# liuQuan98/GCL

Hardware: AMD Instinct MI355X
Metric: active voxels/sec thru ResUNetBN2C fwd+bwd+GCL loss, KITTI 0.3m (higher is better)
Workload: dtype f32; 1 GPU; configs[2]: GCL training step (finest_contrastive_loss), ResUNetBN2C-32 conv1 k=5, KITTI-shaped ray-cast clouds @0.3 m, bs=4 x 7 clouds per GPU, positive groups 'fixed16'; global_batch=4, parallelism=dp1

## Files before the change

gcl_amd/csrc/norm.hip:

```cpp
#include "common.h"

namespace gcl {

static inline int bn_rows_per_wg(long long n, int c) {
  int rows = 1024;
  while (rows > 64 && n / rows < 1024) rows >>= 1;
  (void)c;
  return rows;
}

__device__ __forceinline__ float4 mask_as_y(const unsigned long long* __restrict__ mask, long long e) {
  const unsigned long long* m = mask + (e >> 6) * 4;
  const int b = (int)(e & 63);
  return make_float4((float)((m[0] >> b) & 1), (float)((m[1] >> b) & 1), (float)((m[2] >> b) & 1),
                     (float)((m[3] >> b) & 1));
}

template <bool BWD>
__global__ void __launch_bounds__(256) k_bn_reduce(const float* __restrict__ x, const float* __restrict__ dy,
                                                   const float* __restrict__ y, long long n, int c,
                                                   const float* __restrict__ mean, const float* __restrict__ rstd,
                                                   int relu, const unsigned long long* __restrict__ mask,
                                                   int rows_per_wg, double* partial, int dy_ld = 0, int want_gmax = 0) {
  const long long gld = dy_ld ? dy_ld : c;
  __shared__ double red[2][256][4];
  const int cq_n = c >> 2;
  const int cq = threadIdx.x % cq_n, rl = threadIdx.x / cq_n, rstep = 256 / cq_n;
  const long long r_begin = (long long)blockIdx.x * rows_per_wg;
  long long r_end = r_begin + rows_per_wg;
  if (r_end > n) r_end = n;
  double s0[4] = {0, 0, 0, 0}, s1[4] = {0, 0, 0, 0};
  float gm[4] = {0.f, 0.f, 0.f, 0.f};
  float4 mu = make_float4(0, 0, 0, 0), rs = make_float4(1, 1, 1, 1);
  if (BWD) {
    mu = reinterpret_cast<const float4*>(mean)[cq];
    rs = reinterpret_cast<const float4*>(rstd)[cq];
  }
#define BN_ACC(xv, g, yv)                                                                                     \
  if (!BWD) {                                                                                                 \
    s0[0] += xv.x; s0[1] += xv.y; s0[2] += xv.z; s0[3] += xv.w;                                               \
    s1[0] += (double)xv.x * xv.x; s1[1] += (double)xv.y * xv.y;                                               \
    s1[2] += (double)xv.z * xv.z; s1[3] += (double)xv.w * xv.w;                                               \
  } else {                                                                                                    \
    if (relu) {                                                                                               \
      g.x = yv.x > 0.f ? g.x : 0.f; g.y = yv.y > 0.f ? g.y : 0.f;                                             \
      g.z = yv.z > 0.f ? g.z : 0.f; g.w = yv.w > 0.f ? g.w : 0.f;                                             \
    }                                                                                                         \
    s0[0] += g.x; s0[1] += g.y; s0[2] += g.z; s0[3] += g.w;                                                   \
    gm[0] = fmaxf(gm[0], fabsf(g.x)); gm[1] = fmaxf(gm[1], fabsf(g.y));                                       \
    gm[2] = fmaxf(gm[2], fabsf(g.z)); gm[3] = fmaxf(gm[3], fabsf(g.w));                                       \
    s1[0] += (double)g.x * ((xv.x - mu.x) * rs.x); s1[1] += (double)g.y * ((xv.y - mu.y) * rs.y);             \
    s1[2] += (double)g.z * ((xv.z - mu.z) * rs.z); s1[3] += (double)g.w * ((xv.w - mu.w) * rs.w);             \
  }
  const float4 z4 = make_float4(0, 0, 0, 0);
  long long r = r_begin + rl;
  for (; r + rstep < r_end; r += 2 * rstep) {
    const long long q = r + rstep;
    float4 xa = reinterpret_cast<const float4*>(x + r * c)[cq], xb = reinterpret_cast<const float4*>(x + q * c)[cq];
    float4 ga = z4, gb = z4, ya = z4, yb = z4;
    if (BWD) {
      ga = reinterpret_cast<const float4*>(dy + r * gld)[cq];
      gb = reinterpret_cast<const float4*>(dy + q * gld)[cq];
      if (relu) {
        if (mask) {
          ya = mask_as_y(mask, r * cq_n + cq);
          yb = mask_as_y(mask, q * cq_n + cq);
        } else {
          ya = reinterpret_cast<const float4*>(y + r * c)[cq];
          yb = reinterpret_cast<const float4*>(y + q * c)[cq];
        }
      }
    }
    BN_ACC(xa, ga, ya)
    BN_ACC(xb, gb, yb)
  }
  if (r < r_end) {
    float4 xa = reinterpret_cast<const float4*>(x + r * c)[cq];
    float4 ga = z4, ya = z4;
    if (BWD) {
      ga = reinterpret_cast<const float4*>(dy + r * gld)[cq];
      if (relu) ya = mask ? mask_as_y(mask, r * cq_n + cq) : reinterpret_cast<const float4*>(y + r * c)[cq];
    }
    BN_ACC(xa, ga, ya)
  }
#undef BN_ACC
#pragma unroll
  for (int j = 0; j < 4; ++j) {
    red[0][threadIdx.x][j] = s0[j];
    red[1][threadIdx.x][j] = s1[j];
  }
  __syncthreads();
  if (rl == 0) {
    const long long nwg = gridDim.x;
#pragma unroll
    for (int j = 0; j < 4; ++j) {
      double a = 0, b = 0;
      for (int q = 0; q < rstep; ++q) {
        a += red[0][q * cq_n + cq][j];
        b += red[1][q * cq_n + cq][j];
      }
      partial[(long long)(cq * 4 + j) * nwg + blockIdx.x] = a;
      partial[(long long)(c + cq * 4 + j) * nwg + blockIdx.x] = b;
    }
  }
  if (BWD && want_gmax) {
    __syncthreads();
#pragma unroll
    for (int j = 0; j < 4; ++j) red[0][threadIdx.x][j] = (double)gm[j];
    __syncthreads();
    if (rl == 0) {
      const long long nwg = gridDim.x;
#pragma unroll
      for (int j = 0; j < 4; ++j) {
        double a = 0;
        for (int q = 0; q < rstep; ++q) a = fmax(a, red[0][q * cq_n + cq][j]);
        partial[(long long)(2 * c + cq * 4 + j) * nwg + blockIdx.x] = a;
      }
    }
  }
}

template <typename T>
__device__ __forceinline__ void reduce_runs(const T* __restrict__ p1, const T* __restrict__ p2, int n_part, double& s,
                                            double& ss) {
  __shared__ double red[2][256];
  __shared__ double red2[2][16];
  const int t = threadIdx.x;
  double a0 = 0, a1 = 0, a2 = 0, a3 = 0, b0 = 0, b1 = 0, b2 = 0, b3 = 0;
  int w = t;
  for (; w + 768 < n_part; w += 1024) {
    a0 += (double)p1[w];
    a1 += (double)p1[w + 256];
    a2 += (double)p1[w + 512];
    a3 += (double)p1[w + 768];
    b0 += (double)p2[w];
    b1 += (double)p2[w + 256];
    b2 += (double)p2[w + 512];
    b3 += (double)p2[w + 768];
  }
  for (; w < n_part; w += 256) {
    a0 += (double)p1[w];
    b0 += (double)p2[w];
  }
  red[0][t] = (a0 + a1) + (a2 + a3);
  red[1][t] = (b0 + b1) + (b2 + b3);
  __syncthreads();
  if (t < 32) {
    const int which = t >> 4, g = t & 15;
    double u = 0;
#pragma unroll
    for (int q = 0; q < 16; ++q) u += red[which][g * 16 + q];
    red2[which][g] = u;
  }
  __syncthreads();
  s = 0;
  ss = 0;
  if (t == 0) {
#pragma unroll
    for (int q = 0; q < 16; ++q) {
      s += red2[0][q];
      ss += red2[1][q];
    }
  }
}

__global__ void __launch_bounds__(256) k_bn_stats_final(const double* __restrict__ partial, int nwg, long long n,
                                                        int c, float eps, float momentum, float* running_mean,
                                                        float* running_var, float* mean, float* rstd) {
  const int ch = blockIdx.x;
  double s, ss;
  reduce_runs(partial + (long long)ch * nwg, partial + ((long long)c + ch) * nwg, nwg, s, ss);
  if (threadIdx.x != 0) return;
  double m = s / (double)n;
  double var = ss / (double)n - m * m;
  if (var < 0) var = 0;
  mean[ch] = (float)m;
  rstd[ch] = (float)(1.0 / sqrt(var + (double)eps));
  if (running_mean) {
    double unb = (n > 1) ? var * (double)n / (double)(n - 1) : var;
    running_mean[ch] = (float)((1.0 - momentum) * running_mean[ch] + momentum * m);
    running_var[ch] = (float)((1.0 - momentum) * running_var[ch] + momentum * unb);
  }
}

constexpr int BN_DIRECT_MAX = 1 << 20;
__device__ __forceinline__ void reduce_min_max(const float* __restrict__ p1, const float* __restrict__ p2, int n_part,
                                               float& lo, float& hi) {
  __shared__ float mm[2][256];
  const int t = threadIdx.x;
  float a = 3.0e38f, b = -3.0e38f;
  for (int w = t; w < n_part; w += 256) {
    a = fminf(a, p1[w]);
    b = fmaxf(b, p2[w]);
  }
  mm[0][t] = a;
  mm[1][t] = b;
  __syncthreads();
  for (int o = 128; o > 0; o >>= 1) {
    if (t < o) {
      mm[0][t] = fminf(mm[0][t], mm[0][t + o]);
      mm[1][t] = fmaxf(mm[1][t], mm[1][t + o]);
    }
    __syncthreads();
  }
  lo = mm[0][0];
  hi = mm[1][0];
}

struct BnRange {
  float* xrange;
  const float* weight;
  const float* bias;
  int relu;
  const int* add_amax;
  const int* max_with;
  int* y_amax;
};
__global__ void __launch_bounds__(256) k_bn_stats_direct(const float* __restrict__ partial, int n_part, long long n, int c,
                                                         float eps, float momentum, float* running_mean,
                                                         float* running_var, float* mean, float* rstd, BnRange rg) {
  const int ch = blockIdx.x;
  double s, ss;
  reduce_runs(partial + (long long)ch * n_part, partial + ((long long)c + ch) * n_part, n_part, s, ss);
  float xlo = 0.f, xhi = 0.f;
  if (rg.y_amax)
    reduce_min_max(partial + ((long long)2 * c + ch) * n_part, partial + ((long long)3 * c + ch) * n_part, n_part, xlo, xhi);
  if (threadIdx.x != 0) return;
  double m = s / (double)n;
  double var = ss / (double)n - m * m;
  if (var < 0) var = 0;
  const float mu = (float)m, rs = (float)(1.0 / sqrt(var + (double)eps));
  mean[ch] = mu;
  rstd[ch] = rs;
  if (running_mean) {
    double unb = (n > 1) ? var * (double)n / (double)(n - 1) : var;
    running_mean[ch] = (float)((1.0 - momentum) * running_mean[ch] + momentum * m);
    running_var[ch] = (float)((1.0 - momentum) * running_var[ch] + momentum * unb);
  }
  if (rg.y_amax) {
    if (rg.xrange) {
      rg.xrange[ch] = xlo;
      rg.xrange[c + ch] = xhi;
    }
    const float w = rg.weight[ch], b = rg.bias[ch];
    const float f_lo = (xlo - mu) * rs * w + b, f_hi = (xhi - mu) * rs * w + b;
    float bound = rg.relu ? fmaxf(fmaxf(f_lo, f_hi), 0.f) : fmaxf(fabsf(f_lo), fabsf(f_hi));
    if (rg.add_amax) bound += __int_as_float(amax_slot_bits(rg.add_amax));
    if (rg.max_with) bound = fmaxf(bound, __int_as_float(amax_slot_bits(rg.max_with)));
    amax_slot_publish(rg.y_amax, __float_as_int(bound), (unsigned)ch);
  }
}

struct BnBwdRange {
  const float* xrange;
  const float* mean;
  const float* rstd;
  const float* weight;
  long long n;
  int* dx_amax;
};
__global__ void __launch_bounds__(256) k_bn_bwd_final(const double* __restrict__ partial, int nwg, int c,
                                                      float* sum_g, float* sum_gx, BnBwdRange rg) {
  const int ch = blockIdx.x;
  double s, ss;
  reduce_runs(partial + (long long)ch * nwg, partial + ((long long)c + ch) * nwg, nwg, s, ss);
  double gmax = 0;
  if (rg.dx_amax) {
    __shared__ double gm[256];
    double a = 0;
    const double* p3 = partial + ((long long)2 * c + ch) * nwg;
    for (int w = threadIdx.x; w < nwg; w += 256) a = fmax(a, p3[w]);
    gm[threadIdx.x] = a;
    __syncthreads();
    for (int o = 128; o > 0; o >>= 1) {
      if ((int)threadIdx.x < o) gm[threadIdx.x] = fmax(gm[threadIdx.x], gm[threadIdx.x + o]);
      __syncthreads();
    }
    gmax = gm[0];
  }
  if (threadIdx.x != 0) return;
  sum_g[ch] = (float)s;
  sum_gx[ch] = (float)ss;
  if (rg.dx_amax) {
    const float mu = rg.mean[ch], rs = rg.rstd[ch], inv_n = 1.0f / (float)rg.n;
    const float xh = fmaxf(fabsf(rg.xrange[ch] - mu), fabsf(rg.xrange[c + ch] - mu)) * rs;
    const float bound = fabsf(rg.weight[ch] * rs) * ((float)gmax + fabsf((float)s) * inv_n + xh * fabsf((float)ss) * inv_n);
    amax_slot_publish(rg.dx_amax, __float_as_int(bound * 1.0000153f), (unsigned)ch);
  }
}

__device__ __forceinline__ void publish_amax(float m, int* amax_bits) {
#pragma unroll
  for (int o = 32; o > 0; o >>= 1) m = fmaxf(m, __shfl_xor(m, o));
  __shared__ float wm[4];
  if ((threadIdx.x & 63) == 0) wm[threadIdx.x >> 6] = m;
  __syncthreads();
  if (threadIdx.x == 0) {
    amax_slot_publish(amax_bits, __float_as_int(fmaxf(fmaxf(wm[0], wm[1]), fmaxf(wm[2], wm[3]))), blockIdx.x);
  }
}
__device__ __forceinline__ float amax4(float m, const float4& v) {
  return fmaxf(m, fmaxf(fmaxf(fabsf(v.x), fabsf(v.y)), fmaxf(fabsf(v.z), fabsf(v.w))));
}

struct BnFwdC { float4 mu, rs, wv, bv; };
__device__ __forceinline__ BnFwdC bn_fwd_c(const float* mean, const float* rstd, const float* weight, const float* bias, int cq) {
  BnFwdC k;
  k.mu = reinterpret_cast<const float4*>(mean)[cq]; k.rs = reinterpret_cast<const float4*>(rstd)[cq];
  k.wv = reinterpret_cast<const float4*>(weight)[cq]; k.bv = reinterpret_cast<const float4*>(bias)[cq];
  return k;
}
__device__ __forceinline__ float4 bn_fwd_one(const float4& xv, const float4& rv, bool has_res, int relu, const BnFwdC& k) {
  float4 o;
  o.x = (xv.x - k.mu.x) * k.rs.x * k.wv.x + k.bv.x;
  o.y = (xv.y - k.mu.y) * k.rs.y * k.wv.y + k.bv.y;
  o.z = (xv.z - k.mu.z) * k.rs.z * k.wv.z + k.bv.z;
  o.w = (xv.w - k.mu.w) * k.rs.w * k.wv.w + k.bv.w;
  if (has_res) { o.x += rv.x; o.y += rv.y; o.z += rv.z; o.w += rv.w; }
  if (relu) { o.x = fmaxf(o.x, 0.f); o.y = fmaxf(o.y, 0.f); o.z = fmaxf(o.z, 0.f); o.w = fmaxf(o.w, 0.f); }
  return o;
}
__device__ __forceinline__ void bn_mask_store(unsigned long long* __restrict__ mask, long long e, const float4& o, bool ok) {
  unsigned long long b0 = __ballot(ok && o.x > 0.f), b1 = __ballot(ok && o.y > 0.f), b2 = __ballot(ok && o.z > 0.f),
                     b3 = __ballot(ok && o.w > 0.f);
  if (ok && (threadIdx.x & 63) == 0) {
    unsigned long long* m = mask + (e >> 6) * 4;
    m[0] = b0; m[1] = b1; m[2] = b2; m[3] = b3;
  }
}

template <bool HOIST>
__global__ void __launch_bounds__(256) k_bn_apply(const float* __restrict__ x, long long total4, int c,
                                                  const float* __restrict__ mean, const float* __restrict__ rstd,
                                                  const float* __restrict__ weight, const float* __restrict__ bias,
                                                  const float* __restrict__ residual, int relu,
                                                  float* __restrict__ y, unsigned long long* __restrict__ mask,
                                                  int* amax_bits, int y_ld = 0, unsigned short* __restrict__ planes = nullptr,
                                                  const int* __restrict__ planes_amax = nullptr) {
  const float pscale = planes ? amax_scale(planes_amax) : 1.f;
  const int cq_n = c >> 2;
  const long long S = (long long)gridDim.x * blockDim.x;
  const long long e0 = (long long)blockIdx.x * blockDim.x + threadIdx.x;
  const long long yld4 = (y_ld ? y_ld : c) >> 2;
  const long long rstep = HOIST ? S / cq_n : 0;
  long long row_e = e0 / cq_n;
  const int q0 = (int)(e0 % cq_n);
#define BN_Y(E, ROW) (y_ld ? (HOIST ? reinterpret_cast<float4*>(y)[(ROW)*yld4 + q0]                        \
                                    : reinterpret_cast<float4*>(y)[((E) / cq_n) * yld4 + ((E) % cq_n)])   \
                           : reinterpret_cast<float4*>(y)[E])
  const float4 z4 = make_float4(0, 0, 0, 0);
  float am = 0.f;
  BnFwdC ka, kb;
  if (HOIST) ka = kb = bn_fwd_c(mean, rstd, weight, bias, (int)(e0 % cq_n));
  for (long long e = e0; e - (threadIdx.x & 63) < total4; e += 2 * S) {
    const long long f = e + S;
    const bool oka = e < total4, okb = f < total4;
    if (!HOIST) {
      ka = bn_fwd_c(mean, rstd, weight, bias, (int)((oka ? e : 0) % cq_n));
      kb = bn_fwd_c(mean, rstd, weight, bias, (int)((okb ? f : 0) % cq_n));
    }
    float4 xa = z4, xb = z4, ra = z4, rb = z4;
    if (oka) xa = reinterpret_cast<const float4*>(x)[e];
    if (okb) xb = reinterpret_cast<const float4*>(x)[f];
    if (residual) {
      if (oka) ra = reinterpret_cast<const float4*>(residual)[e];
      if (okb) rb = reinterpret_cast<const float4*>(residual)[f];
    }
    const float4 oa = bn_fwd_one(xa, ra, residual != nullptr, relu, ka);
    const float4 ob = bn_fwd_one(xb, rb, residual != nullptr, relu, kb);
    if (oka) { BN_Y(e, row_e) = oa; am = amax4(am, oa); }
    if (okb) { BN_Y(f, row_e + rstep) = ob; am = amax4(am, ob); }
    if (planes) {
      const long long pld = yld4 * 4;
      if (oka) store_planes4(planes, HOIST ? row_e : e / cq_n, pld, HOIST ? q0 * 4 : (int)(e % cq_n) * 4, oa, pscale);
      if (okb) store_planes4(planes, HOIST ? row_e + rstep : f / cq_n, pld, HOIST ? q0 * 4 : (int)(f % cq_n) * 4, ob, pscale);
    }
    row_e += 2 * rstep;
    if (mask) {
      bn_mask_store(mask, e, oa, oka);
      if (f - (threadIdx.x & 63) < total4) bn_mask_store(mask, f, ob, okb);
    }
  }
#undef BN_Y
  if (amax_bits && !planes) publish_amax(am, amax_bits);
}

struct BnBwdC { float4 mu, rs, wv, sg, sx; };
__device__ __forceinline__ BnBwdC bn_bwd_c(const float* mean, const float* rstd, const float* weight, const float* sum_g,
                                           const float* sum_gx, int cq) {
  BnBwdC k;
  k.mu = reinterpret_cast<const float4*>(mean)[cq]; k.rs = reinterpret_cast<const float4*>(rstd)[cq];
  k.wv = reinterpret_cast<const float4*>(weight)[cq];
  k.sg = reinterpret_cast<const float4*>(sum_g)[cq]; k.sx = reinterpret_cast<const float4*>(sum_gx)[cq];
  return k;
}
__device__ __forceinline__ float4 bn_bwd_one(const float4& xv, const float4& g, float inv_n, const BnBwdC& k) {
  float4 o;
  o.x = k.wv.x * k.rs.x * (g.x - k.sg.x * inv_n - (xv.x - k.mu.x) * k.rs.x * k.sx.x * inv_n);
  o.y = k.wv.y * k.rs.y * (g.y - k.sg.y * inv_n - (xv.y - k.mu.y) * k.rs.y * k.sx.y * inv_n);
  o.z = k.wv.z * k.rs.z * (g.z - k.sg.z * inv_n - (xv.z - k.mu.z) * k.rs.z * k.sx.z * inv_n);
  o.w = k.wv.w * k.rs.w * (g.w - k.sg.w * inv_n - (xv.w - k.mu.w) * k.rs.w * k.sx.w * inv_n);
  return o;
}
__device__ __forceinline__ void relu_gate(float4& g, const float4& yv) {
  g.x = yv.x > 0.f ? g.x : 0.f; g.y = yv.y > 0.f ? g.y : 0.f;
  g.z = yv.z > 0.f ? g.z : 0.f; g.w = yv.w > 0.f ? g.w : 0.f;
}

template <bool HOIST>
__global__ void __launch_bounds__(256) k_bn_bwd_apply(const float* __restrict__ x, const float* __restrict__ dy,
                                                      const float* __restrict__ y, long long total4, int c,
                                                      float inv_n, const float* __restrict__ mean,
                                                      const float* __restrict__ rstd,
                                                      const float* __restrict__ weight,
                                                      const float* __restrict__ sum_g,
                                                      const float* __restrict__ sum_gx, int relu,
                                                      const unsigned long long* __restrict__ mask,
                                                      float* __restrict__ dx, float* __restrict__ dres,
                                                      int* amax_bits, int dy_ld = 0,
                                                      unsigned short* __restrict__ planes = nullptr,
                                                      const int* __restrict__ planes_amax = nullptr) {
  const float pscale = planes ? amax_scale(planes_amax) : 1.f;
  const int cq_n = c >> 2;
  const long long S = (long long)gridDim.x * blockDim.x;
  const long long e0 = (long long)blockIdx.x * blockDim.x + threadIdx.x;
  const long long gld4 = (dy_ld ? dy_ld : c) >> 2;
  const long long rstep = HOIST ? S / cq_n : 0;
  long long row_e = e0 / cq_n;
  const int q0 = (int)(e0 % cq_n);
#define BN_DY(E, ROW) (dy_ld ? (HOIST ? reinterpret_cast<const float4*>(dy)[(ROW)*gld4 + q0]                       \
                                      : reinterpret_cast<const float4*>(dy)[((E) / cq_n) * gld4 + ((E) % cq_n)])  \
                             : reinterpret_cast<const float4*>(dy)[E])
  const float4 z4 = make_float4(0, 0, 0, 0);
  float am = 0.f;
  BnBwdC ka, kb;
  if (HOIST) ka = kb = bn_bwd_c(mean, rstd, weight, sum_g, sum_gx, (int)(e0 % cq_n));
  for (long long e = e0; e < total4; e += 2 * S) {
    const long long f = e + S;
    const bool okb = f < total4;
    if (!HOIST) {
      ka = bn_bwd_c(mean, rstd, weight, sum_g, sum_gx, (int)(e % cq_n));
      kb = bn_bwd_c(mean, rstd, weight, sum_g, sum_gx, (int)((okb ? f : 0) % cq_n));
    }
    float4 xa = reinterpret_cast<const float4*>(x)[e], ga = BN_DY(e, row_e);
    float4 xb = z4, gb = z4, ya = z4, yb = z4;
    if (okb) {
      xb = reinterpret_cast<const float4*>(x)[f];
      gb = BN_DY(f, row_e + rstep);
    }
    row_e += 2 * rstep;
    if (relu) {
      ya = mask ? mask_as_y(mask, e) : reinterpret_cast<const float4*>(y)[e];
      if (okb) yb = mask ? mask_as_y(mask, f) : reinterpret_cast<const float4*>(y)[f];
      relu_gate(ga, ya);
      relu_gate(gb, yb);
    }
    const float4 oa = bn_bwd_one(xa, ga, inv_n, ka);
    reinterpret_cast<float4*>(dx)[e] = oa;
    am = amax4(am, oa);
    if (planes) store_planes4(planes, e / cq_n, c, (int)(e % cq_n) * 4, oa, pscale);
    if (dres) reinterpret_cast<float4*>(dres)[e] = ga;
    if (okb) {
      const float4 ob = bn_bwd_one(xb, gb, inv_n, kb);
      reinterpret_cast<float4*>(dx)[f] = ob;
      am = amax4(am, ob);
      if (planes) store_planes4(planes, f / cq_n, c, (int)(f % cq_n) * 4, ob, pscale);
      if (dres) reinterpret_cast<float4*>(dres)[f] = gb;
    }
  }
#undef BN_DY
  if (amax_bits && !planes) publish_amax(am, amax_bits);
}

template <bool BWD>
__global__ void __launch_bounds__(256) k_row_normalize(const float* __restrict__ a, const float* __restrict__ dy,
                                                       const float* __restrict__ norm_in, long long n, int c,
                                                       float* __restrict__ out, float* __restrict__ norm_out,
                                                       int* out_amax) {
  const int lpr = c >> 2;
  const long long e = (long long)blockIdx.x * blockDim.x + threadIdx.x;
  const long long row = e / lpr;
  const bool ok = row < n;
  float4 v = make_float4(0, 0, 0, 0), g = make_float4(0, 0, 0, 0);
  if (ok) {
    v = reinterpret_cast<const float4*>(a)[e];
    if (BWD) g = reinterpret_cast<const float4*>(dy)[e];
  }
  float s = BWD ? (v.x * g.x + v.y * g.y + v.z * g.z + v.w * g.w) : (v.x * v.x + v.y * v.y + v.z * v.z + v.w * v.w);
  for (int o = 1; o < lpr; o <<= 1) s += __shfl_xor(s, o);
  float m = 0.f;
  if (ok) {
    float4 o4;
    if (!BWD) {
      const float nr = sqrtf(s);
      o4 = make_float4(v.x / nr, v.y / nr, v.z / nr, v.w / nr);
      if ((e % lpr) == 0) norm_out[row] = nr;
    } else {
      const float nr = norm_in[row];
      o4 = make_float4((g.x - v.x * s) / nr, (g.y - v.y * s) / nr, (g.z - v.z * s) / nr, (g.w - v.w * s) / nr);
    }
    reinterpret_cast<float4*>(out)[e] = o4;
    m = amax4(m, o4);
  }
  if (out_amax) publish_amax(m, out_amax);
}

struct SgdPtrs { float* p; const float* g; float* buf; };
__global__ void __launch_bounds__(256) k_sgd_multi(const SgdPtrs* __restrict__ table, const long long* __restrict__ sizes,
                                                   float lr, float momentum, float wd, int first) {
  const SgdPtrs t = table[blockIdx.y];
  const long long n = sizes[blockIdx.y];
  const bool vec = ((((unsigned long long)t.p) | ((unsigned long long)t.g) | ((unsigned long long)t.buf)) & 15ull) == 0;
  const long long n4 = vec ? n / 4 : 0;
  for (long long e = (long long)blockIdx.x * blockDim.x + threadIdx.x; e < n4; e += (long long)gridDim.x * blockDim.x) {
    float4 p = reinterpret_cast<const float4*>(t.p)[e];
    const float4 g = reinterpret_cast<const float4*>(t.g)[e];
    float4 b = make_float4(0, 0, 0, 0);
    if (!first) b = reinterpret_cast<const float4*>(t.buf)[e];
    const float d0 = g.x + wd * p.x, d1 = g.y + wd * p.y, d2 = g.z + wd * p.z, d3 = g.w + wd * p.w;
    b.x = first ? d0 : momentum * b.x + d0;
    b.y = first ? d1 : momentum * b.y + d1;
    b.z = first ? d2 : momentum * b.z + d2;
    b.w = first ? d3 : momentum * b.w + d3;
    reinterpret_cast<float4*>(t.buf)[e] = b;
    p.x -= lr * b.x;
    p.y -= lr * b.y;
    p.z -= lr * b.z;
    p.w -= lr * b.w;
    reinterpret_cast<float4*>(t.p)[e] = p;
  }
  for (long long e = n4 * 4 + (long long)blockIdx.x * blockDim.x + threadIdx.x; e < n; e += (long long)gridDim.x * blockDim.x) {
    const float p = t.p[e];
    const float d = t.g[e] + wd * p;
    const float b = first ? d : momentum * t.buf[e] + d;
    t.buf[e] = b;
    t.p[e] = p - lr * b;
  }
}

static bool bn_c_ok(int c) { return c >= 4 && c % 4 == 0 && (256 % (c / 4)) == 0; }

__global__ void __launch_bounds__(256) k_col_sum_final(const double* __restrict__ partial, int nwg, int c, float* out) {
  const int ch = blockIdx.x;
  double s, ss;
  reduce_runs(partial + (long long)ch * nwg, partial + ((long long)c + ch) * nwg, nwg, s, ss);
  if (threadIdx.x != 0) return;
  out[ch] = (float)s;
}

}

using namespace gcl;

extern "C" {

int64_t gcl_bn_scratch_len(int64_t n, int32_t c) { return cdiv(n, bn_rows_per_wg(n, c)) * 3 * c; }

int gcl_bn_stats(const float* x, int64_t n, int32_t c, float eps, float momentum, float* running_mean,
                 float* running_var, double* scratch, float* mean, float* rstd, void* stream) {
  GCL_CHECK_ARG(x && scratch && mean && rstd, "gcl_bn_stats: null pointer");
  GCL_CHECK_ARG(n > 0 && bn_c_ok(c), "gcl_bn_stats: unsupported shape n=%lld c=%d (c/4 must divide 256)", (long long)n, c);
  hipStream_t st = (hipStream_t)stream;
  const int rows = bn_rows_per_wg(n, c);
  int nwg = (int)cdiv(n, rows);
  hipLaunchKernelGGL(k_bn_reduce<false>, dim3(nwg), dim3(256), 0, st, x, (const float*)nullptr,
                     (const float*)nullptr, (long long)n, c, (const float*)nullptr, (const float*)nullptr, 0,
                     (const unsigned long long*)nullptr, rows, scratch);
  hipLaunchKernelGGL(k_bn_stats_final, dim3((unsigned)c), dim3(256), 0, st, (const double*)scratch, nwg,
                     (long long)n, c, eps, momentum, running_mean, running_var, mean, rstd);
  GCL_CHECK_LAUNCH();
  return GCL_OK;
}

int64_t gcl_bn_tiles_scratch_len(int64_t n_tiles, int32_t c) { (void)n_tiles; return 2 * (int64_t)c; }

int gcl_bn_stats_from_tiles(const float* partial, int64_t n_tiles, int64_t n, int32_t c, float eps, float momentum,
                            float* running_mean, float* running_var, double* scratch, float* mean, float* rstd,
                            void* stream) {
  (void)scratch;
  return gcl_bn_stats_from_tiles_range(partial, n_tiles, n, c, eps, momentum, running_mean, running_var, mean, rstd, nullptr,
                                       nullptr, nullptr, 0, nullptr, nullptr, nullptr, stream);
}

int gcl_bn_stats_from_tiles_range(const float* partial, int64_t n_tiles, int64_t n, int32_t c, float eps, float momentum,
                                  float* running_mean, float* running_var, float* mean, float* rstd, float* xrange,
                                  const float* weight, const float* bias, int32_t relu, const int32_t* add_amax,
                                  const int32_t* max_with, int32_t* y_amax, void* stream) {
  GCL_CHECK_ARG(partial && mean && rstd, "gcl_bn_stats_from_tiles: null pointer");
  GCL_CHECK_ARG(n > 0 && n_tiles > 0 && n_tiles <= BN_DIRECT_MAX && c > 0, "gcl_bn_stats_from_tiles: bad sizes");
  GCL_CHECK_ARG(!y_amax || (weight && bias), "gcl_bn_stats_from_tiles_range: the bound of max|y| needs the BatchNorm's weight and bias");
  const BnRange rg{xrange, weight, bias, relu, (const int*)add_amax, (const int*)max_with, (int*)y_amax};
  hipLaunchKernelGGL(k_bn_stats_direct, dim3((unsigned)c), dim3(256), 0, (hipStream_t)stream, partial, (int)n_tiles,
                     (long long)n, c, eps, momentum, running_mean, running_var, mean, rstd, rg);
  GCL_CHECK_LAUNCH();
  return GCL_OK;
}

int gcl_bn_apply(const float* x, int64_t n, int32_t c, const float* mean, const float* rstd, const float* weight,
                 const float* bias, const float* residual, int32_t relu, float* y, uint64_t* relu_mask,
                 int32_t* y_amax, void* stream) {
  return gcl_bn_apply_ld(x, n, c, mean, rstd, weight, bias, residual, relu, y, 0, relu_mask, y_amax, stream);
}

int gcl_bn_apply_ld(const float* x, int64_t n, int32_t c, const float* mean, const float* rstd, const float* weight,
                    const float* bias, const float* residual, int32_t relu, float* y, int32_t y_ld, uint64_t* relu_mask,
                    int32_t* y_amax, void* stream) {
  return gcl_bn_apply_planes(x, n, c, mean, rstd, weight, bias, residual, relu, y, y_ld, relu_mask, y_amax, nullptr, stream);
}

int gcl_bn_apply_planes(const float* x, int64_t n, int32_t c, const float* mean, const float* rstd, const float* weight,
                        const float* bias, const float* residual, int32_t relu, float* y, int32_t y_ld, uint64_t* relu_mask,
                        int32_t* y_amax, void* planes, void* stream) {
  GCL_CHECK_ARG(x && mean && rstd && weight && bias && y, "gcl_bn_apply: null pointer");
  GCL_CHECK_ARG(n > 0 && c >= 4 && c % 4 == 0, "gcl_bn_apply: unsupported shape");
  GCL_CHECK_ARG(y_ld == 0 || (y_ld >= c && y_ld % 4 == 0), "gcl_bn_apply_ld: y_ld must be 0 or a multiple of 4 >= c");
  GCL_CHECK_ARG(!planes || (y_amax && c % 32 == 0 && (y_ld % 32) == 0),
                "gcl_bn_apply_planes: a plane image needs the slot that holds the bound of max|y| and widths that are multiples of 32");
  long long total4 = n * (c / 4);
  long long g = cdiv(total4, 256);
  if (g > 4096) g = 4096;
  if ((g * 256) % (c / 4) == 0)
    hipLaunchKernelGGL(k_bn_apply<true>, dim3((unsigned)g), dim3(256), 0, (hipStream_t)stream, x, total4, c, mean, rstd,
                       weight, bias, residual, relu, y, (unsigned long long*)(relu ? relu_mask : nullptr), y_amax, y_ld,
                       (unsigned short*)planes, (const int*)y_amax);
  else
    hipLaunchKernelGGL(k_bn_apply<false>, dim3((unsigned)g), dim3(256), 0, (hipStream_t)stream, x, total4, c, mean, rstd,
                       weight, bias, residual, relu, y, (unsigned long long*)(relu ? relu_mask : nullptr), y_amax, y_ld,
                       (unsigned short*)planes, (const int*)y_amax);
  GCL_CHECK_LAUNCH();
  return GCL_OK;
}

int64_t gcl_bn_mask_len(int64_t n, int32_t c) { return cdiv(n * (c / 4), 64) * 4; }

int gcl_bn_bwd_reduce(const float* x, const float* dy, const float* y, const uint64_t* relu_mask, int64_t n,
                      int32_t c, const float* mean, const float* rstd, int32_t relu, double* scratch, float* sum_g,
                      float* sum_gx, void* stream) {
  return gcl_bn_bwd_reduce_ld(x, dy, 0, y, relu_mask, n, c, mean, rstd, relu, scratch, sum_g, sum_gx, stream);
}

int gcl_bn_bwd_reduce_ld(const float* x, const float* dy, int32_t dy_ld, const float* y, const uint64_t* relu_mask, int64_t n,
                         int32_t c, const float* mean, const float* rstd, int32_t relu, double* scratch, float* sum_g,
                         float* sum_gx, void* stream) {
  return gcl_bn_bwd_reduce_range(x, dy, dy_ld, y, relu_mask, n, c, mean, rstd, relu, scratch, sum_g, sum_gx, nullptr, nullptr,
                                 nullptr, stream);
}

int gcl_bn_bwd_reduce_range(const float* x, const float* dy, int32_t dy_ld, const float* y, const uint64_t* relu_mask,
                            int64_t n, int32_t c, const float* mean, const float* rstd, int32_t relu, double* scratch,
                            float* sum_g, float* sum_gx, const float* xrange, const float* weight, int32_t* dx_amax,
                            void* stream) {
  GCL_CHECK_ARG(dy_ld == 0 || (dy_ld >= c && dy_ld % 4 == 0), "gcl_bn_bwd_reduce: dy_ld must be 0 or a multiple of 4 >= c");
  GCL_CHECK_ARG(x && dy && mean && rstd && scratch && sum_g && sum_gx, "gcl_bn_bwd_reduce: null pointer");
  GCL_CHECK_ARG(!relu || y || relu_mask, "gcl_bn_bwd_reduce: y or relu_mask is required when relu is set");
  GCL_CHECK_ARG(n > 0 && bn_c_ok(c), "gcl_bn_bwd_reduce: unsupported shape n=%lld c=%d", (long long)n, c);
  GCL_CHECK_ARG(!dx_amax || (xrange && weight), "gcl_bn_bwd_reduce_range: the bound of max|dx| needs xrange (forward pass) and the weight");
  hipStream_t st = (hipStream_t)stream;
  const int rows = bn_rows_per_wg(n, c);
  int nwg = (int)cdiv(n, rows);
  hipLaunchKernelGGL(k_bn_reduce<true>, dim3(nwg), dim3(256), 0, st, x, dy, y, (long long)n, c, mean, rstd, relu,
                     (const unsigned long long*)relu_mask, rows, scratch, dy_ld, dx_amax ? 1 : 0);
  const BnBwdRange rg{xrange, mean, rstd, weight, (long long)n, (int*)dx_amax};
  hipLaunchKernelGGL(k_bn_bwd_final, dim3((unsigned)c), dim3(256), 0, st, (const double*)scratch, nwg, c,
                     sum_g, sum_gx, rg);
  GCL_CHECK_LAUNCH();
  return GCL_OK;
}

int gcl_bn_bwd_apply(const float* x, const float* dy, const float* y, const uint64_t* relu_mask, int64_t n, int32_t c,
                     const float* mean, const float* rstd, const float* weight, const float* sum_g,
                     const float* sum_gx, int32_t relu, float* dx, float* dres, int32_t* dx_amax, void* stream) {
  return gcl_bn_bwd_apply_ld(x, dy, 0, y, relu_mask, n, c, mean, rstd, weight, sum_g, sum_gx, relu, dx, dres, dx_amax, stream);
}

int gcl_bn_bwd_apply_ld(const float* x, const float* dy, int32_t dy_ld, const float* y, const uint64_t* relu_mask, int64_t n,
                        int32_t c, const float* mean, const float* rstd, const float* weight, const float* sum_g,
                        const float* sum_gx, int32_t relu, float* dx, float* dres, int32_t* dx_amax, void* stream) {
  return gcl_bn_bwd_apply_planes(x, dy, dy_ld, y, relu_mask, n, c, mean, rstd, weight, sum_g, sum_gx, relu, dx, dres, dx_amax,
                                 nullptr, stream);
}

int gcl_bn_bwd_apply_planes(const float* x, const float* dy, int32_t dy_ld, const float* y, const uint64_t* relu_mask, int64_t n,
                            int32_t c, const float* mean, const float* rstd, const float* weight, const float* sum_g,
                            const float* sum_gx, int32_t relu, float* dx, float* dres, int32_t* dx_amax, void* planes,
                            void* stream) {
  GCL_CHECK_ARG(dy_ld == 0 || (dy_ld >= c && dy_ld % 4 == 0), "gcl_bn_bwd_apply: dy_ld must be 0 or a multiple of 4 >= c");
  GCL_CHECK_ARG(x && dy && mean && rstd && weight && sum_g && sum_gx && dx, "gcl_bn_bwd_apply: null pointer");
  GCL_CHECK_ARG(!relu || y || relu_mask, "gcl_bn_bwd_apply: y or relu_mask is required when relu is set");
  GCL_CHECK_ARG(n > 0 && c >= 4 && c % 4 == 0, "gcl_bn_bwd_apply: unsupported shape");
  GCL_CHECK_ARG(!planes || (dx_amax && c % 32 == 0),
                "gcl_bn_bwd_apply_planes: a plane image needs the slot that holds the bound of max|dx| and c a multiple of 32");
  long long total4 = n * (c / 4);
  long long g = cdiv(total4, 256);
  if (g > 4096) g = 4096;
  if ((g * 256) % (c / 4) == 0)
    hipLaunchKernelGGL(k_bn_bwd_apply<true>, dim3((unsigned)g), dim3(256), 0, (hipStream_t)stream, x, dy, y, total4, c,
                       1.0f / (float)n, mean, rstd, weight, sum_g, sum_gx, relu, (const unsigned long long*)relu_mask, dx,
                       dres, dx_amax, dy_ld, (unsigned short*)planes, (const int*)dx_amax);
  else
    hipLaunchKernelGGL(k_bn_bwd_apply<false>, dim3((unsigned)g), dim3(256), 0, (hipStream_t)stream, x, dy, y, total4, c,
                       1.0f / (float)n, mean, rstd, weight, sum_g, sum_gx, relu, (const unsigned long long*)relu_mask, dx,
                       dres, dx_amax, dy_ld, (unsigned short*)planes, (const int*)dx_amax);
  GCL_CHECK_LAUNCH();
  return GCL_OK;
}

static bool rownorm_c_ok(int c) { return c >= 4 && c <= 256 && (c & (c - 1)) == 0; }

int gcl_row_normalize_fwd(const float* x, int64_t n, int32_t c, float* y, float* norm, void* stream) {
  GCL_CHECK_ARG(x && y && norm, "gcl_row_normalize_fwd: null pointer");
  GCL_CHECK_ARG(n > 0 && rownorm_c_ok(c), "gcl_row_normalize_fwd: c must be a power of two in [4, 256] (got %d)", c);
  long long total = n * (c / 4);
  hipLaunchKernelGGL(k_row_normalize<false>, dim3((unsigned)cdiv(total, 256)), dim3(256), 0, (hipStream_t)stream, x,
                     (const float*)nullptr, (const float*)nullptr, (long long)n, c, y, norm, (int*)nullptr);
  GCL_CHECK_LAUNCH();
  return GCL_OK;
}

int gcl_row_normalize_bwd(const float* y, const float* dy, const float* norm, int64_t n, int32_t c, float* dx,
                          int32_t* dx_amax, void* stream) {
  GCL_CHECK_ARG(y && dy && norm && dx, "gcl_row_normalize_bwd: null pointer");
  GCL_CHECK_ARG(n > 0 && rownorm_c_ok(c), "gcl_row_normalize_bwd: c must be a power of two in [4, 256] (got %d)", c);
  long long total = n * (c / 4);
  hipLaunchKernelGGL(k_row_normalize<true>, dim3((unsigned)cdiv(total, 256)), dim3(256), 0, (hipStream_t)stream, y, dy,
                     norm, (long long)n, c, dx, (float*)nullptr, dx_amax);
  GCL_CHECK_LAUNCH();
  return GCL_OK;
}

int gcl_col_sum(const float* x, int64_t n, int32_t c, double* scratch, float* out, void* stream) {
  GCL_CHECK_ARG(x && scratch && out, "gcl_col_sum: null pointer");
  GCL_CHECK_ARG(n > 0 && bn_c_ok(c), "gcl_col_sum: unsupported shape n=%lld c=%d (c/4 must divide 256)", (long long)n, c);
  hipStream_t st = (hipStream_t)stream;
  const int rows = bn_rows_per_wg(n, c);
  int nwg = (int)cdiv(n, rows);
  hipLaunchKernelGGL(k_bn_reduce<false>, dim3(nwg), dim3(256), 0, st, x, (const float*)nullptr,
                     (const float*)nullptr, (long long)n, c, (const float*)nullptr, (const float*)nullptr, 0,
                     (const unsigned long long*)nullptr, rows, scratch);
  hipLaunchKernelGGL(k_col_sum_final, dim3((unsigned)c), dim3(256), 0, st, (const double*)scratch, nwg, c, out);
  GCL_CHECK_LAUNCH();
  return GCL_OK;
}

int gcl_sgd_multi(const void* table, const int64_t* sizes, int32_t n_tensors, float lr, float momentum,
                  float weight_decay, int32_t first, void* stream) {
  GCL_CHECK_ARG(table && sizes && n_tensors > 0 && n_tensors <= 65535, "gcl_sgd_multi: bad argument");
  hipLaunchKernelGGL(k_sgd_multi, dim3(128, (unsigned)n_tensors), dim3(256), 0, (hipStream_t)stream,
                     (const SgdPtrs*)table, (const long long*)sizes, lr, momentum, weight_decay, first);
  GCL_CHECK_LAUNCH();
  return GCL_OK;
}

}
```

Baseline: 46.21 million active voxels/s.

## Rewrite BN reduction as grid-stride loop with buffer loads and wave shuffles

Replaces the per-workgroup contiguous row-block BN reduction with a capped-grid, grid-stride loop over float4 elements, unrolled by four. Out-of-range handling moves to buffer-resource loads, which return zero past the window instead of taking a branch. The ReLU gate is chosen as a template parameter, and the mask is read as whole 64-bit words per wave. The in-block reduction now uses wave shuffles plus a small LDS stage instead of a full 256x4 double LDS reduction, and partial slots are interleaved. The aim is to raise memory-level parallelism, cut partial count, and reduce LDS/branch overhead; it adds a dy_ld limit and relies on buffer-OOB semantics.

```diff
diff --git a/gcl_amd/csrc/norm.hip b/gcl_amd/csrc/norm.hip
--- a/gcl_amd/csrc/norm.hip
+++ b/gcl_amd/csrc/norm.hip
@@ -2,11 +2,14 @@
 
 namespace gcl {
 
-static inline int bn_rows_per_wg(long long n, int c) {
-  int rows = 1024;
-  while (rows > 64 && n / rows < 1024) rows >>= 1;
-  (void)c;
-  return rows;
+constexpr int BN_RED_U = 4;
+constexpr int BN_RED_WGS = 1280;
+static inline int bn_reduce_wgs(long long n, int c) {
+  long long w = cdiv(cdiv(n * (c >> 2), 256), BN_RED_U);
+  if (w > BN_RED_WGS) w = BN_RED_WGS;
+  if (w > n / 64) w = n / 64 > 0 ? n / 64 : 1;
+  if (w > 8) w &= ~7ll;
+  return (int)w;
 }
 
 __device__ __forceinline__ float4 mask_as_y(const unsigned long long* __restrict__ mask, long long e) {
@@ -16,19 +19,31 @@
                      (float)((m[3] >> b) & 1));
 }
 
-template <bool BWD>
+__device__ __forceinline__ __amdgpu_buffer_rsrc_t bn_window(const void* base, long long bytes) {
+  const long long cap = 0x7fffffff;
+  const int records = (int)(bytes < 0 ? 0 : bytes > cap ? cap : bytes);
+  return __builtin_amdgcn_make_buffer_rsrc(const_cast<void*>(base), 0, records, 0x00020000);
+}
+__device__ __forceinline__ float4 bn_window_load(__amdgpu_buffer_rsrc_t w, unsigned byte_off) {
+  typedef unsigned int u32x4 __attribute__((ext_vector_type(4)));
+  const u32x4 v = __builtin_amdgcn_raw_buffer_load_b128(w, (int)byte_off, 0, 0);
+  return make_float4(__uint_as_float(v.x), __uint_as_float(v.y), __uint_as_float(v.z), __uint_as_float(v.w));
+}
+
+template <bool BWD, int GATE>
 __global__ void __launch_bounds__(256) k_bn_reduce(const float* __restrict__ x, const float* __restrict__ dy,
-                                                   const float* __restrict__ y, long long n, int c,
+                                                   const float* __restrict__ y, long long total4, int c,
                                                    const float* __restrict__ mean, const float* __restrict__ rstd,
-                                                   int relu, const unsigned long long* __restrict__ mask,
-                                                   int rows_per_wg, double* partial, int dy_ld = 0, int want_gmax = 0) {
-  const long long gld = dy_ld ? dy_ld : c;
-  __shared__ double red[2][256][4];
-  const int cq_n = c >> 2;
-  const int cq = threadIdx.x % cq_n, rl = threadIdx.x / cq_n, rstep = 256 / cq_n;
-  const long long r_begin = (long long)blockIdx.x * rows_per_wg;
-  long long r_end = r_begin + rows_per_wg;
-  if (r_end > n) r_end = n;
+                                                   const unsigned long long* __restrict__ mask, double* partial,
+                                                   int dy_ld = 0, int want_gmax = 0) {
+  const int cq_n = c >> 2, lg = __ffs(cq_n) - 1;
+  const unsigned lane = threadIdx.x & 63;
+  const int cq = threadIdx.x & (cq_n - 1), wave = __builtin_amdgcn_readfirstlane(threadIdx.x >> 6);
+  const long long S = (long long)gridDim.x * 256;
+  long long ew = (long long)blockIdx.x * 256 + wave * 64;
+  const long long n = total4 >> lg, gld4 = (dy_ld ? dy_ld : c) >> 2, gS = (S >> lg) * gld4;
+  const unsigned cql = ((unsigned)(wave * 64) & (cq_n - 1)) + lane;
+  const unsigned xoff = lane * 16, goff = ((cql >> lg) * (unsigned)gld4 + (unsigned)cq) * 16;
   double s0[4] = {0, 0, 0, 0}, s1[4] = {0, 0, 0, 0};
   float gm[4] = {0.f, 0.f, 0.f, 0.f};
   float4 mu = make_float4(0, 0, 0, 0), rs = make_float4(1, 1, 1, 1);
@@ -36,15 +51,14 @@
     mu = reinterpret_cast<const float4*>(mean)[cq];
     rs = reinterpret_cast<const float4*>(rstd)[cq];
   }
-#define BN_ACC(xv, g, yv)                                                                                     \
+#define BN_ACC(xv, g, on)                                                                                     \
   if (!BWD) {                                                                                                 \
     s0[0] += xv.x; s0[1] += xv.y; s0[2] += xv.z; s0[3] += xv.w;                                               \
     s1[0] += (double)xv.x * xv.x; s1[1] += (double)xv.y * xv.y;                                               \
     s1[2] += (double)xv.z * xv.z; s1[3] += (double)xv.w * xv.w;                                               \
   } else {                                                                                                    \
-    if (relu) {                                                                                               \
-      g.x = yv.x > 0.f ? g.x : 0.f; g.y = yv.y > 0.f ? g.y : 0.f;                                             \
-      g.z = yv.z > 0.f ? g.z : 0.f; g.w = yv.w > 0.f ? g.w : 0.f;                                             \
+    if (GATE) {                                                                                               \
+      g.x = on[0] ? g.x : 0.f; g.y = on[1] ? g.y : 0.f; g.z = on[2] ? g.z : 0.f; g.w = on[3] ? g.w : 0.f;     \
     }                                                                                                         \
     s0[0] += g.x; s0[1] += g.y; s0[2] += g.z; s0[3] += g.w;                                                   \
     gm[0] = fmaxf(gm[0], fabsf(g.x)); gm[1] = fmaxf(gm[1], fabsf(g.y));                                       \
@@ -52,70 +66,69 @@
     s1[0] += (double)g.x * ((xv.x - mu.x) * rs.x); s1[1] += (double)g.y * ((xv.y - mu.y) * rs.y);             \
     s1[2] += (double)g.z * ((xv.z - mu.z) * rs.z); s1[3] += (double)g.w * ((xv.w - mu.w) * rs.w);             \
   }
-  const float4 z4 = make_float4(0, 0, 0, 0);
-  long long r = r_begin + rl;
-  for (; r + rstep < r_end; r += 2 * rstep) {
-    const long long q = r + rstep;
-    float4 xa = reinterpret_cast<const float4*>(x + r * c)[cq], xb = reinterpret_cast<const float4*>(x + q * c)[cq];
-    float4 ga = z4, gb = z4, ya = z4, yb = z4;
-    if (BWD) {
-      ga = reinterpret_cast<const float4*>(dy + r * gld)[cq];
-      gb = reinterpret_cast<const float4*>(dy + q * gld)[cq];
-      if (relu) {
-        if (mask) {
-          ya = mask_as_y(mask, r * cq_n + cq);
-          yb = mask_as_y(mask, q * cq_n + cq);
-        } else {
-          ya = reinterpret_cast<const float4*>(y + r * c)[cq];
-          yb = reinterpret_cast<const float4*>(y + q * c)[cq];
-        }
+  for (; ew < total4; ew += BN_RED_U * S) {
+    float4 xv[BN_RED_U], gv[BN_RED_U], yv[BN_RED_U];
+    unsigned long long mw[BN_RED_U][4];
+#pragma unroll
+    for (int j = 0; j < BN_RED_U; ++j) {
+      const long long ej = ew + j * S, rj = ej >> lg;
+      xv[j] = bn_window_load(bn_window(reinterpret_cast<const float4*>(x) + ej, (total4 - ej) * 16), xoff);
+      gv[j] = yv[j] = make_float4(0, 0, 0, 0);
+      mw[j][0] = mw[j][1] = mw[j][2] = mw[j][3] = 0;
+      if (BWD)
+        gv[j] = bn_window_load(bn_window(reinterpret_cast<const float4*>(dy) + rj * gld4, ((n - 1 - rj) * gld4 + cq_n) * 16), goff);
+      if (GATE == 2) yv[j] = bn_window_load(bn_window(reinterpret_cast<const float4*>(y) + ej, (total4 - ej) * 16), xoff);
+      if (GATE == 1 && ej < total4) {
+        const unsigned long long* m = mask + (ej >> 6) * 4;
+        mw[j][0] = m[0]; mw[j][1] = m[1]; mw[j][2] = m[2]; mw[j][3] = m[3];
       }
     }
-    BN_ACC(xa, ga, ya)
-    BN_ACC(xb, gb, yb)
-  }
-  if (r < r_end) {
-    float4 xa = reinterpret_cast<const float4*>(x + r * c)[cq];
-    float4 ga = z4, ya = z4;
-    if (BWD) {
-      ga = reinterpret_cast<const float4*>(dy + r * gld)[cq];
-      if (relu) ya = mask ? mask_as_y(mask, r * cq_n + cq) : reinterpret_cast<const float4*>(y + r * c)[cq];
-    }
-    BN_ACC(xa, ga, ya)
+#pragma unroll
+    for (int j = 0; j < BN_RED_U; ++j) {
+      const bool on[4] = {GATE == 1 ? (bool)((mw[j][0] >> lane) & 1) : yv[j].x > 0.f,
+                          GATE == 1 ? (bool)((mw[j][1] >> lane) & 1) : yv[j].y > 0.f,
+                          GATE == 1 ? (bool)((mw[j][2] >> lane) & 1) : yv[j].z > 0.f,
+                          GATE == 1 ? (bool)((mw[j][3] >> lane) & 1) : yv[j].w > 0.f};
+      BN_ACC(xv[j], gv[j], on)
+    }
   }
 #undef BN_ACC
-#pragma unroll
-  for (int j = 0; j < 4; ++j) {
-    red[0][threadIdx.x][j] = s0[j];
-    red[1][threadIdx.x][j] = s1[j];
+  for (int o = 32; o >= cq_n; o >>= 1) {
+#pragma unroll
+    for (int j = 0; j < 4; ++j) {
+      s0[j] += __shfl_xor(s0[j], o);
+      s1[j] += __shfl_xor(s1[j], o);
+      if (BWD) gm[j] = fmaxf(gm[j], __shfl_xor(gm[j], o));
+    }
+  }
+  __shared__ double red[3][8][64];
+  __shared__ float redm[3][4][64];
+  const int nown = cq_n > 64 ? cq_n >> 6 : 1;
+  if (wave >= nown) {
+#pragma unroll
+    for (int j = 0; j < 4; ++j) {
+      red[wave - nown][j][lane] = s0[j];
+      red[wave - nown][4 + j][lane] = s1[j];
+      if (BWD) redm[wave - nown][j][lane] = gm[j];
+    }
   }
   __syncthreads();
-  if (rl == 0) {
+  if (wave < nown && (int)lane < cq_n) {
+    for (int w = wave + nown; w < 4; w += nown) {
+#pragma unroll
+      for (int j = 0; j < 4; ++j) {
+        s0[j] += red[w - nown][j][lane];
+        s1[j] += red[w - nown][4 + j][lane];
+        if (BWD) gm[j] = fmaxf(gm[j], redm[w - nown][j][lane]);
+      }
+    }
     const long long nwg = gridDim.x;
+    const long long slot = (nwg & 7) == 0 ? (long long)(blockIdx.x & 7) * (nwg >> 3) + (blockIdx.x >> 3) : blockIdx.x;
 #pragma unroll
     for (int j = 0; j < 4; ++j) {
-      double a = 0, b = 0;
-      for (int q = 0; q < rstep; ++q) {
-        a += red[0][q * cq_n + cq][j];
-        b += red[1][q * cq_n + cq][j];
-      }
-      partial[(long long)(cq * 4 + j) * nwg + blockIdx.x] = a;
-      partial[(long long)(c + cq * 4 + j) * nwg + blockIdx.x] = b;
-    }
-  }
-  if (BWD && want_gmax) {
-    __syncthreads();
-#pragma unroll
-    for (int j = 0; j < 4; ++j) red[0][threadIdx.x][j] = (double)gm[j];
-    __syncthreads();
-    if (rl == 0) {
-      const long long nwg = gridDim.x;
-#pragma unroll
-      for (int j = 0; j < 4; ++j) {
-        double a = 0;
-        for (int q = 0; q < rstep; ++q) a = fmax(a, red[0][q * cq_n + cq][j]);
-        partial[(long long)(2 * c + cq * 4 + j) * nwg + blockIdx.x] = a;
-      }
+      partial[(long long)(cq * 4 + j) * nwg + slot] = s0[j];
+      partial[(long long)(c + cq * 4 + j) * nwg + slot] = s1[j];
+      if (BWD && want_gmax) partial[(long long)(2 * c + cq * 4 + j) * nwg + slot] = (double)gm[j];
     }
   }
 }
@@ -554,18 +567,17 @@
 
 extern "C" {
 
-int64_t gcl_bn_scratch_len(int64_t n, int32_t c) { return cdiv(n, bn_rows_per_wg(n, c)) * 3 * c; }
+int64_t gcl_bn_scratch_len(int64_t n, int32_t c) { return (int64_t)bn_reduce_wgs(n, c) * 3 * c; }
 
 int gcl_bn_stats(const float* x, int64_t n, int32_t c, float eps, float momentum, float* running_mean,
                  float* running_var, double* scratch, float* mean, float* rstd, void* stream) {
   GCL_CHECK_ARG(x && scratch && mean && rstd, "gcl_bn_stats: null pointer");
   GCL_CHECK_ARG(n > 0 && bn_c_ok(c), "gcl_bn_stats: unsupported shape n=%lld c=%d (c/4 must divide 256)", (long long)n, c);
   hipStream_t st = (hipStream_t)stream;
-  const int rows = bn_rows_per_wg(n, c);
-  int nwg = (int)cdiv(n, rows);
-  hipLaunchKernelGGL(k_bn_reduce<false>, dim3(nwg), dim3(256), 0, st, x, (const float*)nullptr,
-                     (const float*)nullptr, (long long)n, c, (const float*)nullptr, (const float*)nullptr, 0,
-                     (const unsigned long long*)nullptr, rows, scratch);
+  const int nwg = bn_reduce_wgs(n, c);
+  hipLaunchKernelGGL((k_bn_reduce<false, 0>), dim3(nwg), dim3(256), 0, st, x, (const float*)nullptr,
+                     (const float*)nullptr, (long long)n * (c >> 2), c, (const float*)nullptr, (const float*)nullptr,
+                     (const unsigned long long*)nullptr, scratch);
   hipLaunchKernelGGL(k_bn_stats_final, dim3((unsigned)c), dim3(256), 0, st, (const double*)scratch, nwg,
                      (long long)n, c, eps, momentum, running_mean, running_var, mean, rstd);
   GCL_CHECK_LAUNCH();
@@ -651,15 +663,16 @@
                             float* sum_g, float* sum_gx, const float* xrange, const float* weight, int32_t* dx_amax,
                             void* stream) {
   GCL_CHECK_ARG(dy_ld == 0 || (dy_ld >= c && dy_ld % 4 == 0), "gcl_bn_bwd_reduce: dy_ld must be 0 or a multiple of 4 >= c");
+  GCL_CHECK_ARG(dy_ld <= (1 << 20), "gcl_bn_bwd_reduce: dy_ld above 2^20 (a lane's 32-bit offset spans 64 rows of dy)");
   GCL_CHECK_ARG(x && dy && mean && rstd && scratch && sum_g && sum_gx, "gcl_bn_bwd_reduce: null pointer");
   GCL_CHECK_ARG(!relu || y || relu_mask, "gcl_bn_bwd_reduce: y or relu_mask is required when relu is set");
   GCL_CHECK_ARG(n > 0 && bn_c_ok(c), "gcl_bn_bwd_reduce: unsupported shape n=%lld c=%d", (long long)n, c);
   GCL_CHECK_ARG(!dx_amax || (xrange && weight), "gcl_bn_bwd_reduce_range: the bound of max|dx| needs xrange (forward pass) and the weight");
   hipStream_t st = (hipStream_t)stream;
-  const int rows = bn_rows_per_wg(n, c);
-  int nwg = (int)cdiv(n, rows);
-  hipLaunchKernelGGL(k_bn_reduce<true>, dim3(nwg), dim3(256), 0, st, x, dy, y, (long long)n, c, mean, rstd, relu,
-                     (const unsigned long long*)relu_mask, rows, scratch, dy_ld, dx_amax ? 1 : 0);
+  const int nwg = bn_reduce_wgs(n, c);
+  auto* kernel = !relu ? k_bn_reduce<true, 0> : relu_mask ? k_bn_reduce<true, 1> : k_bn_reduce<true, 2>;
+  hipLaunchKernelGGL(kernel, dim3(nwg), dim3(256), 0, st, x, dy, y, (long long)n * (c >> 2), c, mean, rstd,
+                     (const unsigned long long*)relu_mask, scratch, dy_ld, dx_amax ? 1 : 0);
   const BnBwdRange rg{xrange, mean, rstd, weight, (long long)n, (int*)dx_amax};
   hipLaunchKernelGGL(k_bn_bwd_final, dim3((unsigned)c), dim3(256), 0, st, (const double*)scratch, nwg, c,
                      sum_g, sum_gx, rg);
@@ -732,11 +745,10 @@
   GCL_CHECK_ARG(x && scratch && out, "gcl_col_sum: null pointer");
   GCL_CHECK_ARG(n > 0 && bn_c_ok(c), "gcl_col_sum: unsupported shape n=%lld c=%d (c/4 must divide 256)", (long long)n, c);
   hipStream_t st = (hipStream_t)stream;
-  const int rows = bn_rows_per_wg(n, c);
-  int nwg = (int)cdiv(n, rows);
-  hipLaunchKernelGGL(k_bn_reduce<false>, dim3(nwg), dim3(256), 0, st, x, (const float*)nullptr,
-                     (const float*)nullptr, (long long)n, c, (const float*)nullptr, (const float*)nullptr, 0,
-                     (const unsigned long long*)nullptr, rows, scratch);
+  const int nwg = bn_reduce_wgs(n, c);
+  hipLaunchKernelGGL((k_bn_reduce<false, 0>), dim3(nwg), dim3(256), 0, st, x, (const float*)nullptr,
+                     (const float*)nullptr, (long long)n * (c >> 2), c, (const float*)nullptr, (const float*)nullptr,
+                     (const unsigned long long*)nullptr, scratch);
   hipLaunchKernelGGL(k_col_sum_final, dim3((unsigned)c), dim3(256), 0, st, (const double*)scratch, nwg, c, out);
   GCL_CHECK_LAUNCH();
   return GCL_OK;
```

Result: no change. 46.21 million active voxels/s (-0.0%).
